# jianfenglihg/Unsupervised_depth_OpticalFlow_egomotion

Hardware: AMD Instinct MI355X
Metric: frame-pairs/sec (832x256, geom mode) (higher is better)
Workload: dtype f32; 1 GPU; train_step: mode=geom, 832x256, batch=4/GPU, num_scales=3, fwd+bwd+Adam; global_batch=4, parallelism=dp1, hw_queues=4, stream_priorities=auto

## Files before the change

### unsupervised_depth_opticalflow_egomotion_amd/csrc/ops_wino.hip

```cpp
#include "dfe_internal.h"
#include "dfe_mfma_stage.h"
#include "dfe_device.h"
#include <hip/hip_runtime.h>
#include <algorithm>
#include <cstdlib>

namespace dfe {


struct WinoEpi { const float* bias; float slope; float* y2; long y2bs; };
__device__ __forceinline__ float wino_act(float v, float bv, float slope) { v += bv; return v > 0.0f ? v : v * slope; }

#ifndef WINO_SCHED
#define WINO_SCHED 1
#endif
constexpr int WN_CC = 16;
constexpr int WN_XP = 20;

template <bool TRANSPOSED>
__device__ __forceinline__ void wino_weight_one(const float* __restrict__ w, float* __restrict__ U, int K, int C, int Kpad, int idx) {
  const int k = idx % Kpad, c = idx / Kpad;
  float g[9];
#pragma unroll
  for (int t = 0; t < 9; ++t) {
    float v = 0.0f;
    if (k < K) v = TRANSPOSED ? w[(static_cast<long>(c) * K + k) * 9 + 8 - t] : w[(static_cast<long>(k) * C + c) * 9 + t];
    g[t] = v;
  }
  float r[4][3];
#pragma unroll
  for (int j = 0; j < 3; ++j) {
    r[0][j] = g[j];
    r[1][j] = 0.5f * ((g[j] + g[3 + j]) + g[6 + j]);
    r[2][j] = 0.5f * ((g[j] - g[3 + j]) + g[6 + j]);
    r[3][j] = g[6 + j];
  }
  float* o = U + ((static_cast<long>(k >> 5) * C + c) * 32 + (k & 31)) * 16;
#pragma unroll
  for (int i = 0; i < 4; ++i) {
    o[i * 4 + 0] = r[i][0];
    o[i * 4 + 1] = 0.5f * ((r[i][0] + r[i][1]) + r[i][2]);
    o[i * 4 + 2] = 0.5f * ((r[i][0] - r[i][1]) + r[i][2]);
    o[i * 4 + 3] = r[i][2];
  }
}

template <bool TRANSPOSED>
__global__ void __launch_bounds__(256) k_wino_weights(const float* __restrict__ w, float* __restrict__ U, int K, int C, int Kpad) {
  const int idx = blockIdx.x * 256 + threadIdx.x;
  if (idx >= Kpad * C) return;
  wino_weight_one<TRANSPOSED>(w, U, K, C, Kpad, idx);
}

__global__ void __launch_bounds__(256) k_wino_weights_multi(const long* __restrict__ table, const int* __restrict__ blockmap) {
  const long* e = table + 6L * blockmap[blockIdx.x];
  const float* w = reinterpret_cast<const float*>(e[0]);
  float* U = reinterpret_cast<float*>(e[1]);
  const int K = static_cast<int>(e[2]), C = static_cast<int>(e[3]), Kpad = (K + 31) / 32 * 32;
  const int idx = (static_cast<int>(blockIdx.x) - static_cast<int>(e[5])) * 256 + threadIdx.x;
  if (idx >= Kpad * C) return;
  if (e[4]) wino_weight_one<true>(w, U, K, C, Kpad, idx);
  else wino_weight_one<false>(w, U, K, C, Kpad, idx);
}

__global__ void __launch_bounds__(256) k_wino_sum(const float* __restrict__ part, float* __restrict__ y, long ybs, int nsp, int B, long KHW,
                                                  long HWo, WinoEpi epi) {
  const long idx = static_cast<long>(blockIdx.x) * 256 + threadIdx.x;
  if (idx >= B * KHW) return;
  float s = part[idx];
  for (int k = 1; k < nsp; ++k) s += part[static_cast<long>(k) * B * KHW + idx];
  const long b = idx / KHW, r = idx - b * KHW;
  if (epi.bias || epi.slope != 1.0f) s = wino_act(s, epi.bias ? epi.bias[r / HWo] : 0.0f, epi.slope);
  y[b * ybs + r] = s;
  if (epi.y2) epi.y2[b * epi.y2bs + r] = s;
}

template <int PP, int NW, int NH>
__global__ void __launch_bounds__(64 * NW, 2) k_wino_fwd16(const float* __restrict__ x, const float* __restrict__ U, float* __restrict__ y,
                                                       long ybs, int B, int C, int K, int H, int W, int P, int TH, int TW, int ntiles,
                                                       unsigned nkt, int dil, unsigned nsp, int cps, float* __restrict__ part, WinoEpi epi,
                                                       unsigned nitems) {
  extern __shared__ float lds[];
  const int tid = threadIdx.x, lane = tid & 63, wv = tid >> 6, n = lane & 15, kq = lane >> 4;
  for (unsigned item = blockIdx.x; item < nitems; item += gridDim.x) {
  if (item != blockIdx.x) __syncthreads();
  const unsigned lid = xcd_swizzle(item, nitems);
  const int kt = static_cast<int>(lid % nkt), sp = static_cast<int>((lid / nkt) % nsp), tb = static_cast<int>(lid / (nkt * nsp));
  const int cbeg = sp * cps, Cend = min(C, cbeg + cps);
  const int Ho = H + 2 * P - 2, Wo = W + 2 * P - 2, HW = H * W;
  const int tile = min(tb * (16 * NW) + wv * 16 + n, ntiles - 1);
  int b, ty, tx, py = 0, px = 0;
  if (PP >= 0 || dil == 1) {
    b = tile / (TH * TW);
    const int tr = tile - b * TH * TW;
    ty = tr / TW; tx = tr - ty * TW;
  } else {
    const int per_row = TW * dil, per_phase = TH * per_row, per_img = per_phase * dil;
    b = tile / per_img;
    int tr = tile - b * per_img;
    py = tr / per_phase; tr -= py * per_phase;
    ty = tr / per_row; tr -= ty * per_row;
    tx = tr / dil; px = tr - tx * dil;
  }
  const int iy0 = 2 * ty - P, ix0 = 2 * tx - P;
  constexpr bool PAIR = PP >= 0;
  constexpr bool USE_L = PP == 1 || PP == 2, USE_R = PP == 1 || PP == 0;
  unsigned off[16], inb = 0;
  bool edge_l = false, edge_r = false;
  if (PAIR) {
    const bool okL = tx >= 1, okR = 2 * tx + 3 < W, okO = 2 * tx + 1 < W;
    edge_l = USE_L && okL && n == 0;
    edge_r = USE_R && okR && (n == 15 || tx == TW - 1);
#pragma unroll
    for (int i = 0; i < 4; ++i) {
      const int yy = iy0 + i;
      const bool ok = yy >= 0 && yy < H;
      const unsigned rowb = 4u * (static_cast<unsigned>(b) * C * HW + (ok ? yy * W : 0));
      off[i] = rowb + (okO ? 8u * static_cast<unsigned>(tx) : 0u);
      off[4 + i] = rowb + (edge_l ? 8u * static_cast<unsigned>(tx - 1) : edge_r ? 8u * static_cast<unsigned>(tx + 1) : 0u);
      off[8 + i] = 0; off[12 + i] = 0;
      inb |= ok ? (1u << i) : 0u;
    }
    inb |= (okL ? 16u : 0u) | (okR ? 32u : 0u) | (okO ? 64u : 0u);
  } else {
    const int Hq = H / dil, Wq = W / dil;
#pragma unroll
    for (int i = 0; i < 4; ++i)
#pragma unroll
      for (int j = 0; j < 4; ++j) {
        const int yy = iy0 + i, xx = ix0 + j;
        const bool ok = yy >= 0 && yy < Hq && xx >= 0 && xx < Wq;
        off[i * 4 + j] = 4u * (static_cast<unsigned>(b) * C * HW + (ok ? (py + dil * yy) * W + px + dil * xx : 0));
        inb |= ok ? (1u << (i * 4 + j)) : 0u;
      }
  }
  f32x4 acc[NH][16];
#pragma unroll
  for (int h = 0; h < NH; ++h)
#pragma unroll
    for (int s = 0; s < 16; ++s) acc[h][s] = f32x4{0.0f, 0.0f, 0.0f, 0.0f};
  const float* Ut = U + static_cast<long>(kt) * C * 512;
  const char* xc = reinterpret_cast<const char*>(x);
  float dn[16];
  unsigned mn;

  unsigned cbl = 4u * static_cast<unsigned>(cbeg + kq) * HW;
  const unsigned cstep = 16u * static_cast<unsigned>(HW);
  auto issue = [&](int c) {
    const bool cok = c < Cend;
    mn = cok ? inb : 0u;
    const unsigned cb = cok ? cbl : 0u;
    cbl += cstep;
    if (PAIR) {
#pragma unroll
      for (int i = 0; i < 4; ++i) {
        const f32x2 p = *reinterpret_cast<const f32x2*>(xc + (off[i] + cb));
        dn[2 * i] = p[0]; dn[2 * i + 1] = p[1];
      }
      if (edge_l || edge_r) {
#pragma unroll
        for (int i = 0; i < 4; ++i) {
          const f32x2 p = *reinterpret_cast<const f32x2*>(xc + (off[4 + i] + cb));
          dn[8 + 2 * i] = p[0]; dn[9 + 2 * i] = p[1];
        }
      }
    } else {
#pragma unroll
      for (int q = 0; q < 16; ++q) dn[q] = *reinterpret_cast<const float*>(xc + (off[q] + cb));
    }
  };
  auto shr1 = [](float v) { return __int_as_float(__builtin_amdgcn_update_dpp(0, __float_as_int(v), 0x111, 0xF, 0xF, true)); };
  auto shl1 = [](float v) { return __int_as_float(__builtin_amdgcn_update_dpp(0, __float_as_int(v), 0x101, 0xF, 0xF, true)); };
  constexpr unsigned NEED = 0xFu | (USE_L ? 16u : 0u) | (USE_R ? 32u : 0u) | 64u;
  const bool plain_wave = PAIR && __all(static_cast<int>((inb & NEED) == NEED)) != 0;
  auto gather = [&](float (&d)[16]) {
    if (PAIR && plain_wave && __all(static_cast<int>(mn != 0u)) != 0) {
#pragma unroll
      for (int i = 0; i < 4; ++i) {
        const float o1 = dn[2 * i], o2 = dn[2 * i + 1], e1 = dn[8 + 2 * i], e2 = dn[9 + 2 * i];
        float l1 = 0.0f, l2 = 0.0f, r1 = 0.0f, r2 = 0.0f;
        if (USE_L) {
          if (PP == 2) { l1 = shr1(o1); l1 = edge_l ? e1 : l1; }
          l2 = shr1(o2); l2 = edge_l ? e2 : l2;
        }
        if (USE_R) {
          r1 = shl1(o1); r1 = edge_r ? e1 : r1;
          if (PP == 0) { r2 = shl1(o2); r2 = edge_r ? e2 : r2; }
        }
        if (PP == 1) { d[4 * i] = l2; d[4 * i + 1] = o1; d[4 * i + 2] = o2; d[4 * i + 3] = r1; }
        else if (PP == 0) { d[4 * i] = o1; d[4 * i + 1] = o2; d[4 * i + 2] = r1; d[4 * i + 3] = r2; }
        else { d[4 * i] = l1; d[4 * i + 1] = l2; d[4 * i + 2] = o1; d[4 * i + 3] = o2; }
      }
    } else if (PAIR) {
#pragma unroll
      for (int i = 0; i < 4; ++i) {
        const bool rok = (mn >> i) & 1u;
        const bool oko = rok && (mn & 64u);
        const float o1 = oko ? dn[2 * i] : 0.0f, o2 = oko ? dn[2 * i + 1] : 0.0f;
        const float e1 = rok ? dn[8 + 2 * i] : 0.0f, e2 = rok ? dn[9 + 2 * i] : 0.0f;
        float l1 = 0.0f, l2 = 0.0f, r1 = 0.0f, r2 = 0.0f;
        if (USE_L) {
          if (PP == 2) l1 = shr1(o1);
          l2 = shr1(o2);
          if (PP == 2) l1 = (mn & 16u) ? (edge_l ? e1 : l1) : 0.0f;
          l2 = (mn & 16u) ? (edge_l ? e2 : l2) : 0.0f;
        }
        if (USE_R) {
          r1 = shl1(o1);
          if (PP == 0) r2 = shl1(o2);
          r1 = (mn & 32u) ? (edge_r ? e1 : r1) : 0.0f;
          if (PP == 0) r2 = (mn & 32u) ? (edge_r ? e2 : r2) : 0.0f;
        }
        if (PP == 1) { d[4 * i] = l2; d[4 * i + 1] = o1; d[4 * i + 2] = o2; d[4 * i + 3] = r1; }
        else if (PP == 0) { d[4 * i] = o1; d[4 * i + 1] = o2; d[4 * i + 2] = r1; d[4 * i + 3] = r2; }
        else { d[4 * i] = l1; d[4 * i + 1] = l2; d[4 * i + 2] = o1; d[4 * i + 3] = o2; }
      }
    } else {
#pragma unroll
      for (int q = 0; q < 16; ++q) d[q] = ((mn >> q) & 1u) ? dn[q] : 0.0f;
    }
  };
#pragma unroll
  for (int i = 8; i < 16; ++i) dn[i] = 0.0f;
  issue(cbeg + kq);
  constexpr int SC = 8, SLAB = SC * 32 * WN_XP;
  constexpr int NTH = 64 * NW;
  f32x4 wreg[SC * 128 / NTH];
  auto wfetch = [&](int c0) {
    const int nc = min(SC, Cend - c0);
#pragma unroll
    for (int i = 0; i < SC * 128 / NTH; ++i) {
      const int e = tid + i * NTH;
      wreg[i] = *reinterpret_cast<const f32x4*>(Ut + static_cast<long>(c0) * 512 + (e < nc * 128 ? e : 0) * 4);
    }
  };
  auto wstore = [&](float* buf) {
#pragma unroll
    for (int i = 0; i < SC * 128 / NTH; ++i) {
      const int e = tid + i * NTH;
      *reinterpret_cast<f32x4*>(buf + (e >> 2) * WN_XP + (e & 3) * 4) = wreg[i];
    }
  };
  wfetch(cbeg);
  wstore(lds);
  __syncthreads();
  int cur = 0;
  for (int c0 = cbeg; c0 < Cend; c0 += SC) {
    const int nc = min(SC, Cend - c0);
    const bool more = c0 + SC < Cend;
    if (more) wfetch(c0 + SC);
    const float* slab = lds + cur * SLAB;
    for (int cs = 0; cs < nc; cs += 4) {
      float d[16], t[16], v[16];
      const float* up = slab + (min(cs + kq, nc - 1) * 32 + n) * WN_XP;
      auto ldU = [&](int h, int q) { return *reinterpret_cast<const f32x4*>(up + h * 16 * WN_XP + 4 * q); };
      f32x4 ua, ub, uc;
      if (NH == 2 && WINO_SCHED) { ua = ldU(0, 0); ub = ldU(0, 1); __builtin_amdgcn_sched_barrier(0); }
      gather(d);
      issue(c0 + cs + 4 + kq);
#pragma unroll
      for (int j = 0; j < 4; ++j) {
        t[j] = d[j] - d[8 + j];
        t[4 + j] = d[4 + j] + d[8 + j];
        t[8 + j] = d[8 + j] - d[4 + j];
        t[12 + j] = d[4 + j] - d[12 + j];
      }
#pragma unroll
      for (int i = 0; i < 4; ++i) {
        v[i * 4 + 0] = t[i * 4] - t[i * 4 + 2];
        v[i * 4 + 1] = t[i * 4 + 1] + t[i * 4 + 2];
        v[i * 4 + 2] = t[i * 4 + 2] - t[i * 4 + 1];
        v[i * 4 + 3] = t[i * 4 + 1] - t[i * 4 + 3];
      }
      if (NH == 2 && WINO_SCHED) {
        auto mfma4 = [&](int h, int q, const f32x4& u) {
#pragma unroll
          for (int j = 0; j < 4; ++j) acc[h][4 * q + j] = __builtin_amdgcn_mfma_f32_16x16x4f32(u[j], v[4 * q + j], acc[h][4 * q + j], 0, 0, 0);
        };
        __builtin_amdgcn_sched_barrier(0);
        uc = ldU(0, 2);
        mfma4(0, 0, ua); ua = ldU(0, 3);
        mfma4(0, 1, ub); ub = ldU(1, 0);
        mfma4(0, 2, uc); uc = ldU(1, 1);
        mfma4(0, 3, ua); ua = ldU(1, 2);
        mfma4(1, 0, ub); ub = ldU(1, 3);
        mfma4(1, 1, uc);
        mfma4(1, 2, ua);
        mfma4(1, 3, ub);
#define SGB_DS(n) __builtin_amdgcn_sched_group_barrier(0x100, n, 0)
#define SGB_MFMA(n) __builtin_amdgcn_sched_group_barrier(0x008, n, 0)
        SGB_DS(1); SGB_MFMA(4); SGB_DS(1); SGB_MFMA(4); SGB_DS(1); SGB_MFMA(4); SGB_DS(1); SGB_MFMA(4); SGB_DS(1); SGB_MFMA(4); SGB_DS(1); SGB_MFMA(12);
#undef SGB_DS
#undef SGB_MFMA
        __builtin_amdgcn_sched_barrier(0);
        continue;
      }
#pragma unroll
      for (int h = 0; h < NH; ++h) {
        float u[16];
#pragma unroll
        for (int q = 0; q < 4; ++q) {
          const f32x4 w4 = *reinterpret_cast<const f32x4*>(up + h * 16 * WN_XP + 4 * q);
          u[4 * q] = w4[0]; u[4 * q + 1] = w4[1]; u[4 * q + 2] = w4[2]; u[4 * q + 3] = w4[3];
        }
#pragma unroll
        for (int s = 0; s < 16; ++s) acc[h][s] = __builtin_amdgcn_mfma_f32_16x16x4f32(u[s], v[s], acc[h][s], 0, 0, 0);
      }
    }
    if (more) {
      wstore(lds + (cur ^ 1) * SLAB);
      __syncthreads();
      cur ^= 1;
    }
  }
  if (tb * (16 * NW) + wv * 16 + n >= ntiles) continue;
  const int Hoq = (PP >= 0 || dil == 1) ? Ho : H / dil, Woq = (PP >= 0 || dil == 1) ? Wo : W / dil;
  const int oy = 2 * ty, ox = 2 * tx;
  const int sy = dil * Wo, sx = dil;
  const long kplane = static_cast<long>(Ho) * Wo;
  const long ooff = static_cast<long>(py + dil * oy) * Wo + px + dil * ox;
  float* yb = (nsp > 1 ? part + (static_cast<long>(sp) * B + b) * K * kplane : y + b * ybs) + ooff;
  const bool fused = nsp == 1 && (epi.bias != nullptr || epi.slope != 1.0f);
  float* y2b = (nsp == 1 && epi.y2) ? epi.y2 + b * epi.y2bs + ooff : nullptr;
  const bool even_w = dil == 1 && (Wo & 1) == 0;
  const bool pair_st = even_w && (reinterpret_cast<uintptr_t>(nsp > 1 ? part : y) & 7) == 0 && ((nsp > 1 ? 0 : ybs) & 1) == 0;
  const bool pair_st2 = even_w && y2b && (reinterpret_cast<uintptr_t>(epi.y2) & 7) == 0 && (epi.y2bs & 1) == 0;
#pragma unroll
  for (int h = 0; h < NH; ++h)
#pragma unroll
    for (int r = 0; r < 4; ++r) {
      const int k = kt * 32 + 16 * h + 4 * kq + r;
      if (k >= K) continue;
      float t0[4], t1[4];
#pragma unroll
      for (int s = 0; s < 4; ++s) {
        t0[s] = (acc[h][s][r] + acc[h][4 + s][r]) + acc[h][8 + s][r];
        t1[s] = (acc[h][4 + s][r] - acc[h][8 + s][r]) - acc[h][12 + s][r];
      }
      float y00 = (t0[0] + t0[1]) + t0[2], y01 = (t0[1] - t0[2]) - t0[3];
      float y10 = (t1[0] + t1[1]) + t1[2], y11 = (t1[1] - t1[2]) - t1[3];
      if (fused) {
        const float bv = epi.bias ? epi.bias[k] : 0.0f;
        y00 = wino_act(y00, bv, epi.slope); y01 = wino_act(y01, bv, epi.slope);
        y10 = wino_act(y10, bv, epi.slope); y11 = wino_act(y11, bv, epi.slope);
      }
      float* o = yb + static_cast<long>(k) * Ho * Wo;
      if (pair_st) {
        if (ox < Woq) {
          if (oy < Hoq) *reinterpret_cast<f32x2*>(o) = f32x2{y00, y01};
          if (oy + 1 < Hoq) *reinterpret_cast<f32x2*>(o + sy) = f32x2{y10, y11};
        }
      } else {
        if (oy < Hoq) {
          if (ox < Woq) o[0] = y00;
          if (ox + 1 < Woq) o[sx] = y01;
        }
        if (oy + 1 < Hoq) {
          if (ox < Woq) o[sy] = y10;
          if (ox + 1 < Woq) o[sy + sx] = y11;
        }
      }
      if (y2b) {
        float* o2 = y2b + static_cast<long>(k) * Ho * Wo;
        if (pair_st2) {
          if (ox < Woq) {
            if (oy < Hoq) *reinterpret_cast<f32x2*>(o2) = f32x2{y00, y01};
            if (oy + 1 < Hoq) *reinterpret_cast<f32x2*>(o2 + sy) = f32x2{y10, y11};
          }
        } else {
          if (oy < Hoq) {
            if (ox < Woq) o2[0] = y00;
            if (ox + 1 < Woq) o2[sx] = y01;
          }
          if (oy + 1 < Hoq) {
            if (ox < Woq) o2[sy] = y10;
            if (ox + 1 < Woq) o2[sy + sx] = y11;
          }
        }
      }
    }
  }
}

}

using namespace dfe;

static int wn_dims(int B, int Ci, int Co, int H, int W, int P) {
  if (B <= 0 || Ci <= 0 || Co <= 0 || H <= 0 || W <= 0) return DFE_ERR_DIMS;
  if (P < 0 || P > 2) return DFE_ERR_UNSUPPORTED;
  if (H + 2 * P < 3 || W + 2 * P < 3) return DFE_ERR_DIMS;
  if (static_cast<long>(B) * Ci * H * W >= (1L << 30) || static_cast<long>(Co) * H * W >= (1L << 31) || Co > 65535 * 32) return DFE_ERR_DIMS;
  return DFE_OK;
}

extern "C" long dfe_wino_weight_floats(int Ci, int Co) { return (Ci <= 0 || Co <= 0) ? 0 : static_cast<long>((Co + 31) / 32) * 32 * Ci * 16; }

extern "C" long dfe_wino_weight_floats(int Ci, int Co);

struct WinoSplit { int nsp, cps; long part_floats; };

static WinoSplit wino_split(long ntiles, int Kpad, int Ci, int B, int Co, int Ho, int Wo) {
  WinoSplit w{1, Ci, 0};
  static const bool enabled = env_int("DFE_WINO_SPLIT", 1) != 0;
  const long nblk = (ntiles + 63) / 64 * (Kpad / 32);
  if (!enabled || nblk >= 384 || Ci < 64) return w;
  int nsp = static_cast<int>((512 + nblk - 1) / nblk);
  nsp = std::min(nsp, std::min(Ci / 32, 8));
  if (nsp < 2) return w;
  w.cps = ((Ci + nsp - 1) / nsp + 7) / 8 * 8;
  w.nsp = (Ci + w.cps - 1) / w.cps;
  if (w.nsp < 2) { w.nsp = 1; w.cps = Ci; return w; }
  w.part_floats = static_cast<long>(w.nsp) * B * Co * Ho * Wo;
  return w;
}

static int wino_run(const float* x, const float* weight, float* y, long y_batch_stride, float* wbuf, float* part, long part_floats, int B,
                    int Ci, int Co, int H, int W, int P, int dil, int transposed_weight, void* stream, WinoEpi epi = WinoEpi{nullptr, 1.0f, nullptr, 0}) {
  if (!x || !y || !wbuf) return DFE_ERR_NULL;
  const int rc = wn_dims(B, Ci, Co, H, W, P);
  if (rc != DFE_OK) return rc;
  if (dil < 1 || (dil > 1 && (P != 1 || H % dil != 0 || W % dil != 0 || H / dil < 2 || W / dil < 2))) return DFE_ERR_UNSUPPORTED;
  const int Ho = dil > 1 ? H : H + 2 * P - 2, Wo = dil > 1 ? W : W + 2 * P - 2;
  if (y_batch_stride < static_cast<long>(Co) * Ho * Wo || (epi.y2 && epi.y2bs < static_cast<long>(Co) * Ho * Wo)) return DFE_ERR_DIMS;
  if ((reinterpret_cast<uintptr_t>(wbuf) & 15) != 0) return DFE_ERR_UNSUPPORTED;
  if (part && (reinterpret_cast<uintptr_t>(part) & 15) != 0) return DFE_ERR_UNSUPPORTED;
  hipStream_t st = static_cast<hipStream_t>(stream);
  const int Kpad = (Co + 31) / 32 * 32;
  const int nw = Kpad * Ci;
  if (weight) {
    if (transposed_weight) k_wino_weights<true><<<(nw + 255) / 256, 256, 0, st>>>(weight, wbuf, Co, Ci, Kpad);
    else k_wino_weights<false><<<(nw + 255) / 256, 256, 0, st>>>(weight, wbuf, Co, Ci, Kpad);
    DFE_LAUNCH_CHECK();
  }
  const int TH = (Ho / dil + 1) / 2, TW = (Wo / dil + 1) / 2;
  const long ntiles = static_cast<long>(B) * TH * TW * dil * dil;
  if (ntiles >= (1L << 31)) return DFE_ERR_DIMS;
  const size_t lds_bytes = sizeof(float) * WN_CC * 32 * WN_XP;
  {
    const unsigned nkt = Kpad / 32;
    WinoSplit sp = wino_split(ntiles, Kpad, Ci, B, Co, Ho, Wo);
    if (dil > 1 || !part || part_floats < sp.part_floats) sp = WinoSplit{1, Ci, 0};
    const int tpb = 64;
    const long nblk = (ntiles + tpb - 1) / tpb * nkt * sp.nsp;
    if (nblk >= (1L << 31)) return DFE_ERR_DIMS;
    static const bool pair_ok = env_int("DFE_WINO_PAIR", 1) != 0;
    const bool pair = pair_ok && dil == 1 && W % 2 == 0 && (reinterpret_cast<uintptr_t>(x) & 7) == 0;
    const unsigned nitems = static_cast<unsigned>(nblk);
    static const int persist = env_int("DFE_WINO_PERSIST", 0);
    const unsigned g = persist > 0 ? std::min(nitems, static_cast<unsigned>(persist)) : nitems;
    const int nt = static_cast<int>(ntiles);
    const int pp = pair ? P : -1;
#define WN_LAUNCH(PPV, NHV) k_wino_fwd16<PPV, 4, NHV><<<g, 256, lds_bytes, st>>>(x, wbuf, y, y_batch_stride, B, Ci, Co, H, W, P, TH, TW, nt, nkt, dil, static_cast<unsigned>(sp.nsp), sp.cps, part, epi, nitems)
    if (Co <= 16) {
      if (pp == 1) WN_LAUNCH(1, 1); else if (pp == 0) WN_LAUNCH(0, 1); else if (pp == 2) WN_LAUNCH(2, 1); else WN_LAUNCH(-1, 1);
    } else {
      if (pp == 1) WN_LAUNCH(1, 2); else if (pp == 0) WN_LAUNCH(0, 2); else if (pp == 2) WN_LAUNCH(2, 2); else WN_LAUNCH(-1, 2);
    }
#undef WN_LAUNCH
    DFE_LAUNCH_CHECK();
    if (sp.nsp > 1) {
      const long khw = static_cast<long>(Co) * Ho * Wo, n = B * khw;
      k_wino_sum<<<static_cast<unsigned>((n + 255) / 256), 256, 0, st>>>(part, y, y_batch_stride, sp.nsp, B, khw, static_cast<long>(Ho) * Wo, epi);
    }
  }
  DFE_LAUNCH_CHECK();
  return DFE_OK;
}

extern "C" long dfe_wino_scratch_floats(int B, int Ci, int Co, int H, int W, int P) {
  if (B <= 0 || Ci <= 0 || Co <= 0 || H <= 0 || W <= 0 || P < 0 || P > 2) return 0;
  const int Ho = H + 2 * P - 2, Wo = W + 2 * P - 2;
  if (Ho < 1 || Wo < 1) return 0;
  const int Kpad = (Co + 31) / 32 * 32;
  const long ntiles = static_cast<long>(B) * ((Ho + 1) / 2) * ((Wo + 1) / 2);
  return static_cast<long>(Kpad) * Ci * 16 + wino_split(ntiles, Kpad, Ci, B, Co, Ho, Wo).part_floats;
}

extern "C" int dfe_wino_conv3x3(const float* x, const float* weight, float* y, long y_batch_stride, float* wbuf, long wbuf_floats, int B,
                                int Ci, int Co, int H, int W, int P, int transposed_weight, void* stream) {
  if (!weight) return DFE_ERR_NULL;
  const long ufl = dfe_wino_weight_floats(Ci, Co);
  if (wbuf_floats < ufl) return DFE_ERR_WORKSPACE;
  return wino_run(x, weight, y, y_batch_stride, wbuf, wbuf ? wbuf + ufl : nullptr, wbuf_floats - ufl, B, Ci, Co, H, W, P, 1, transposed_weight, stream);
}

extern "C" int dfe_wino_conv3x3_dilated(const float* x, const float* weight, float* y, long y_batch_stride, float* wbuf, int B,
                                        int Ci, int Co, int H, int W, int dilation, int transposed_weight, void* stream) {
  if (!weight) return DFE_ERR_NULL;
  return wino_run(x, weight, y, y_batch_stride, wbuf, nullptr, 0, B, Ci, Co, H, W, 1, dilation, transposed_weight, stream);
}

extern "C" int dfe_wino_conv3x3_u(const float* x, const float* U, float* y, long y_batch_stride, float* part, long part_floats, int B, int Ci,
                                  int Co, int H, int W, int P, int dilation, void* stream) {
  return wino_run(x, nullptr, y, y_batch_stride, const_cast<float*>(U), part, part_floats, B, Ci, Co, H, W, dilation > 1 ? 1 : P, dilation, 0,
                  stream);
}

extern "C" int dfe_wino_conv3x3_u_act(const float* x, const float* U, const float* bias, float slope, float* y, long y_batch_stride, float* y2,
                                      long y2_batch_stride, float* part, long part_floats, int B, int Ci, int Co, int H, int W, int P,
                                      int dilation, void* stream) {
  return wino_run(x, nullptr, y, y_batch_stride, const_cast<float*>(U), part, part_floats, B, Ci, Co, H, W, dilation > 1 ? 1 : P, dilation, 0,
                  stream, WinoEpi{bias, slope, y2, y2_batch_stride});
}

extern "C" long dfe_wino_transform_blocks(int Ci, int Co) {
  if (Ci <= 0 || Co <= 0) return 0;
  return (static_cast<long>((Co + 31) / 32 * 32) * Ci + 255) / 256;
}

extern "C" int dfe_wino_transform_weights_multi(const long* table, const int* blockmap, int n_blocks, void* stream) {
  if (!table || !blockmap) return DFE_ERR_NULL;
  if (n_blocks <= 0) return DFE_ERR_DIMS;
  k_wino_weights_multi<<<n_blocks, 256, 0, static_cast<hipStream_t>(stream)>>>(table, blockmap);
  DFE_LAUNCH_CHECK();
  return DFE_OK;
}
```

Before: 434.1 frame-pairs/s.

## Use buffer loads with OOB offsets and restructure Winograd channel loop pipeline

Replaces global loads in the Winograd forward kernel with raw buffer loads whose out-of-bounds offsets (a sentinel value) return zero in hardware, removing the per-element mask selects in the gather. The edge/zero handling via DPP now uses the old-value operand, and a wave-uniform 'inner' flag skips fixups for interior waves. The channel loop is restructured into a two-step-per-slab software pipeline with explicit placement of the next input load and LDS weight store between the transform halves. It adds complexity and relies on buffer OOB semantics, and it tightens the dimension limit accordingly.

```diff
diff --git a/unsupervised_depth_opticalflow_egomotion_amd/csrc/ops_wino.hip b/unsupervised_depth_opticalflow_egomotion_amd/csrc/ops_wino.hip
--- a/unsupervised_depth_opticalflow_egomotion_amd/csrc/ops_wino.hip
+++ b/unsupervised_depth_opticalflow_egomotion_amd/csrc/ops_wino.hip
@@ -16,6 +16,8 @@
 #endif
 constexpr int WN_CC = 16;
 constexpr int WN_XP = 20;
+constexpr unsigned WN_OOB = 0xfffffff0u;
+typedef unsigned u32x2 __attribute__((ext_vector_type(2)));
 
 template <bool TRANSPOSED>
 __device__ __forceinline__ void wino_weight_one(const float* __restrict__ w, float* __restrict__ U, int K, int C, int Kpad, int idx) {
@@ -82,6 +84,7 @@
                                                        unsigned nitems) {
   extern __shared__ float lds[];
   const int tid = threadIdx.x, lane = tid & 63, wv = tid >> 6, n = lane & 15, kq = lane >> 4;
+  const float* up0 = lds + (kq * 32 + n) * WN_XP;
   for (unsigned item = blockIdx.x; item < nitems; item += gridDim.x) {
   if (item != blockIdx.x) __syncthreads();
   const unsigned lid = xcd_swizzle(item, nitems);
@@ -105,23 +108,24 @@
   const int iy0 = 2 * ty - P, ix0 = 2 * tx - P;
   constexpr bool PAIR = PP >= 0;
   constexpr bool USE_L = PP == 1 || PP == 2, USE_R = PP == 1 || PP == 0;
-  unsigned off[16], inb = 0;
-  bool edge_l = false, edge_r = false;
+  constexpr int NV = PAIR ? 8 : 16;
+  unsigned vo[NV];
+  bool zl = false, zr = false;
+  const unsigned lane0 = 4u * (static_cast<unsigned>(b) * C + kq) * HW;
   if (PAIR) {
     const bool okL = tx >= 1, okR = 2 * tx + 3 < W, okO = 2 * tx + 1 < W;
-    edge_l = USE_L && okL && n == 0;
-    edge_r = USE_R && okR && (n == 15 || tx == TW - 1);
+    const bool edge_l = USE_L && okL && n == 0;
+    const bool edge_r = USE_R && okR && (n == 15 || tx == TW - 1);
+    zl = USE_L && !okL && n != 0;
+    zr = USE_R && n != 15 && (PP == 0 ? edge_r : !okR);
 #pragma unroll
     for (int i = 0; i < 4; ++i) {
       const int yy = iy0 + i;
       const bool ok = yy >= 0 && yy < H;
-      const unsigned rowb = 4u * (static_cast<unsigned>(b) * C * HW + (ok ? yy * W : 0));
-      off[i] = rowb + (okO ? 8u * static_cast<unsigned>(tx) : 0u);
-      off[4 + i] = rowb + (edge_l ? 8u * static_cast<unsigned>(tx - 1) : edge_r ? 8u * static_cast<unsigned>(tx + 1) : 0u);
-      off[8 + i] = 0; off[12 + i] = 0;
-      inb |= ok ? (1u << i) : 0u;
-    }
-    inb |= (okL ? 16u : 0u) | (okR ? 32u : 0u) | (okO ? 64u : 0u);
+      const unsigned rowb = lane0 + 4u * static_cast<unsigned>(ok ? yy * W : 0);
+      vo[i] = ok && okO ? rowb + 8u * static_cast<unsigned>(tx) : WN_OOB;
+      vo[4 + i] = ok && edge_l ? rowb + 8u * static_cast<unsigned>(tx - 1) : ok && edge_r ? rowb + 8u * static_cast<unsigned>(tx + 1) : WN_OOB;
+    }
   } else {
     const int Hq = H / dil, Wq = W / dil;
 #pragma unroll
@@ -130,99 +134,90 @@
       for (int j = 0; j < 4; ++j) {
         const int yy = iy0 + i, xx = ix0 + j;
         const bool ok = yy >= 0 && yy < Hq && xx >= 0 && xx < Wq;
-        off[i * 4 + j] = 4u * (static_cast<unsigned>(b) * C * HW + (ok ? (py + dil * yy) * W + px + dil * xx : 0));
-        inb |= ok ? (1u << (i * 4 + j)) : 0u;
-      }
-  }
+        vo[i * 4 + j] = ok ? lane0 + 4u * static_cast<unsigned>((py + dil * yy) * W + px + dil * xx) : WN_OOB;
+      }
+  }
+  const int inner = PAIR ? __builtin_amdgcn_readfirstlane(static_cast<int>(__builtin_amdgcn_ballot_w64(zl || zr) != 0ull)) : 0;
   f32x4 acc[NH][16];
 #pragma unroll
   for (int h = 0; h < NH; ++h)
 #pragma unroll
     for (int s = 0; s < 16; ++s) acc[h][s] = f32x4{0.0f, 0.0f, 0.0f, 0.0f};
   const float* Ut = U + static_cast<long>(kt) * C * 512;
-  const char* xc = reinterpret_cast<const char*>(x);
+  const int ns = (Cend - cbeg + 3) >> 2;
   float dn[16];
-  unsigned mn;
-
-  unsigned cbl = 4u * static_cast<unsigned>(cbeg + kq) * HW;
-  const unsigned cstep = 16u * static_cast<unsigned>(HW);
-  auto issue = [&](int c) {
-    const bool cok = c < Cend;
-    mn = cok ? inb : 0u;
-    const unsigned cb = cok ? cbl : 0u;
-    cbl += cstep;
+
+  const char* xs = reinterpret_cast<const char*>(x) + 4L * cbeg * HW;
+  const long cstep = 16L * HW;
+  const int nrec = static_cast<int>(4u * static_cast<unsigned>(B) * C * HW);
+  const bool past = cbeg + 4 * (ns - 1) + kq >= Cend;
+  auto issue = [&](bool last) {
+    const __amdgpu_buffer_rsrc_t xr = __builtin_amdgcn_make_buffer_rsrc(const_cast<char*>(xs), 0, nrec, 0x00020000);
+    xs += cstep;
+    auto loads = [&]() {
+      if (PAIR) {
+#pragma unroll
+        for (int q = 0; q < 8; ++q) {
+          const u32x2 p = __builtin_amdgcn_raw_buffer_load_b64(xr, vo[q], 0, 0);
+          dn[2 * q] = __uint_as_float(p[0]); dn[2 * q + 1] = __uint_as_float(p[1]);
+        }
+      } else {
+#pragma unroll
+        for (int q = 0; q < 16; ++q) dn[q] = __uint_as_float(__builtin_amdgcn_raw_buffer_load_b32(xr, vo[q], 0, 0));
+      }
+    };
+    if (last) {
+#pragma unroll
+      for (int q = 0; q < 16; ++q) dn[q] = 0.0f;
+      if (!past) loads();
+    } else {
+      loads();
+    }
+  };
+  auto shr1 = [](float old, float v) { return __int_as_float(__builtin_amdgcn_update_dpp(__float_as_int(old), __float_as_int(v), 0x111, 0xF, 0xF, false)); };
+  auto shl1 = [](float old, float v) { return __int_as_float(__builtin_amdgcn_update_dpp(__float_as_int(old), __float_as_int(v), 0x101, 0xF, 0xF, false)); };
+  auto gather = [&](float (&d)[16]) {
     if (PAIR) {
-#pragma unroll
-      for (int i = 0; i < 4; ++i) {
-        const f32x2 p = *reinterpret_cast<const f32x2*>(xc + (off[i] + cb));
-        dn[2 * i] = p[0]; dn[2 * i + 1] = p[1];
-      }
-      if (edge_l || edge_r) {
-#pragma unroll
-        for (int i = 0; i < 4; ++i) {
-          const f32x2 p = *reinterpret_cast<const f32x2*>(xc + (off[4 + i] + cb));
-          dn[8 + 2 * i] = p[0]; dn[9 + 2 * i] = p[1];
-        }
-      }
-    } else {
-#pragma unroll
-      for (int q = 0; q < 16; ++q) dn[q] = *reinterpret_cast<const float*>(xc + (off[q] + cb));
-    }
-  };
-  auto shr1 = [](float v) { return __int_as_float(__builtin_amdgcn_update_dpp(0, __float_as_int(v), 0x111, 0xF, 0xF, true)); };
-  auto shl1 = [](float v) { return __int_as_float(__builtin_amdgcn_update_dpp(0, __float_as_int(v), 0x101, 0xF, 0xF, true)); };
-  constexpr unsigned NEED = 0xFu | (USE_L ? 16u : 0u) | (USE_R ? 32u : 0u) | 64u;
-  const bool plain_wave = PAIR && __all(static_cast<int>((inb & NEED) == NEED)) != 0;
-  auto gather = [&](float (&d)[16]) {
-    if (PAIR && plain_wave && __all(static_cast<int>(mn != 0u)) != 0) {
+      float l1[4], l2[4], r1[4], r2[4], k1[4], k2[4];
 #pragma unroll
       for (int i = 0; i < 4; ++i) {
         const float o1 = dn[2 * i], o2 = dn[2 * i + 1], e1 = dn[8 + 2 * i], e2 = dn[9 + 2 * i];
-        float l1 = 0.0f, l2 = 0.0f, r1 = 0.0f, r2 = 0.0f;
+        l1[i] = l2[i] = r1[i] = r2[i] = 0.0f;
+        k1[i] = PP == 0 ? e1 : 0.0f; k2[i] = PP == 0 ? e2 : 0.0f;
         if (USE_L) {
-          if (PP == 2) { l1 = shr1(o1); l1 = edge_l ? e1 : l1; }
-          l2 = shr1(o2); l2 = edge_l ? e2 : l2;
+          if (PP == 2) l1[i] = shr1(e1, o1);
+          l2[i] = shr1(e2, o2);
         }
         if (USE_R) {
-          r1 = shl1(o1); r1 = edge_r ? e1 : r1;
-          if (PP == 0) { r2 = shl1(o2); r2 = edge_r ? e2 : r2; }
-        }
-        if (PP == 1) { d[4 * i] = l2; d[4 * i + 1] = o1; d[4 * i + 2] = o2; d[4 * i + 3] = r1; }
-        else if (PP == 0) { d[4 * i] = o1; d[4 * i + 1] = o2; d[4 * i + 2] = r1; d[4 * i + 3] = r2; }
-        else { d[4 * i] = l1; d[4 * i + 1] = l2; d[4 * i + 2] = o1; d[4 * i + 3] = o2; }
-      }
-    } else if (PAIR) {
+          r1[i] = shl1(e1, o1);
+          if (PP == 0) r2[i] = shl1(e2, o2);
+        }
+      }
+      if (inner) {
+#pragma unroll
+        for (int i = 0; i < 4; ++i) {
+          if (USE_L) {
+            if (PP == 2) l1[i] = zl ? 0.0f : l1[i];
+            l2[i] = zl ? 0.0f : l2[i];
+          }
+          if (USE_R) {
+            r1[i] = zr ? k1[i] : r1[i];
+            if (PP == 0) r2[i] = zr ? k2[i] : r2[i];
+          }
+        }
+      }
 #pragma unroll
       for (int i = 0; i < 4; ++i) {
-        const bool rok = (mn >> i) & 1u;
-        const bool oko = rok && (mn & 64u);
-        const float o1 = oko ? dn[2 * i] : 0.0f, o2 = oko ? dn[2 * i + 1] : 0.0f;
-        const float e1 = rok ? dn[8 + 2 * i] : 0.0f, e2 = rok ? dn[9 + 2 * i] : 0.0f;
-        float l1 = 0.0f, l2 = 0.0f, r1 = 0.0f, r2 = 0.0f;
-        if (USE_L) {
-          if (PP == 2) l1 = shr1(o1);
-          l2 = shr1(o2);
-          if (PP == 2) l1 = (mn & 16u) ? (edge_l ? e1 : l1) : 0.0f;
-          l2 = (mn & 16u) ? (edge_l ? e2 : l2) : 0.0f;
-        }
-        if (USE_R) {
-          r1 = shl1(o1);
-          if (PP == 0) r2 = shl1(o2);
-          r1 = (mn & 32u) ? (edge_r ? e1 : r1) : 0.0f;
-          if (PP == 0) r2 = (mn & 32u) ? (edge_r ? e2 : r2) : 0.0f;
-        }
-        if (PP == 1) { d[4 * i] = l2; d[4 * i + 1] = o1; d[4 * i + 2] = o2; d[4 * i + 3] = r1; }
-        else if (PP == 0) { d[4 * i] = o1; d[4 * i + 1] = o2; d[4 * i + 2] = r1; d[4 * i + 3] = r2; }
-        else { d[4 * i] = l1; d[4 * i + 1] = l2; d[4 * i + 2] = o1; d[4 * i + 3] = o2; }
+        const float o1 = dn[2 * i], o2 = dn[2 * i + 1];
+        if (PP == 1) { d[4 * i] = l2[i]; d[4 * i + 1] = o1; d[4 * i + 2] = o2; d[4 * i + 3] = r1[i]; }
+        else if (PP == 0) { d[4 * i] = o1; d[4 * i + 1] = o2; d[4 * i + 2] = r1[i]; d[4 * i + 3] = r2[i]; }
+        else { d[4 * i] = l1[i]; d[4 * i + 1] = l2[i]; d[4 * i + 2] = o1; d[4 * i + 3] = o2; }
       }
     } else {
 #pragma unroll
-      for (int q = 0; q < 16; ++q) d[q] = ((mn >> q) & 1u) ? dn[q] : 0.0f;
+      for (int q = 0; q < 16; ++q) d[q] = dn[q];
     }
   };
-#pragma unroll
-  for (int i = 8; i < 16; ++i) dn[i] = 0.0f;
-  issue(cbeg + kq);
   constexpr int SC = 8, SLAB = SC * 32 * WN_XP;
   constexpr int NTH = 64 * NW;
   f32x4 wreg[SC * 128 / NTH];
@@ -241,74 +236,88 @@
       *reinterpret_cast<f32x4*>(buf + (e >> 2) * WN_XP + (e & 3) * 4) = wreg[i];
     }
   };
-  wfetch(cbeg);
-  wstore(lds);
-  __syncthreads();
-  int cur = 0;
-  for (int c0 = cbeg; c0 < Cend; c0 += SC) {
-    const int nc = min(SC, Cend - c0);
-    const bool more = c0 + SC < Cend;
-    if (more) wfetch(c0 + SC);
-    const float* slab = lds + cur * SLAB;
-    for (int cs = 0; cs < nc; cs += 4) {
-      float d[16], t[16], v[16];
-      const float* up = slab + (min(cs + kq, nc - 1) * 32 + n) * WN_XP;
-      auto ldU = [&](int h, int q) { return *reinterpret_cast<const f32x4*>(up + h * 16 * WN_XP + 4 * q); };
-      f32x4 ua, ub, uc;
-      if (NH == 2 && WINO_SCHED) { ua = ldU(0, 0); ub = ldU(0, 1); __builtin_amdgcn_sched_barrier(0); }
-      gather(d);
-      issue(c0 + cs + 4 + kq);
-#pragma unroll
-      for (int j = 0; j < 4; ++j) {
-        t[j] = d[j] - d[8 + j];
-        t[4 + j] = d[4 + j] + d[8 + j];
-        t[8 + j] = d[8 + j] - d[4 + j];
-        t[12 + j] = d[4 + j] - d[12 + j];
-      }
-#pragma unroll
-      for (int i = 0; i < 4; ++i) {
-        v[i * 4 + 0] = t[i * 4] - t[i * 4 + 2];
-        v[i * 4 + 1] = t[i * 4 + 1] + t[i * 4 + 2];
-        v[i * 4 + 2] = t[i * 4 + 2] - t[i * 4 + 1];
-        v[i * 4 + 3] = t[i * 4 + 1] - t[i * 4 + 3];
-      }
-      if (NH == 2 && WINO_SCHED) {
-        auto mfma4 = [&](int h, int q, const f32x4& u) {
-#pragma unroll
-          for (int j = 0; j < 4; ++j) acc[h][4 * q + j] = __builtin_amdgcn_mfma_f32_16x16x4f32(u[j], v[4 * q + j], acc[h][4 * q + j], 0, 0, 0);
-        };
-        __builtin_amdgcn_sched_barrier(0);
-        uc = ldU(0, 2);
-        mfma4(0, 0, ua); ua = ldU(0, 3);
-        mfma4(0, 1, ub); ub = ldU(1, 0);
-        mfma4(0, 2, uc); uc = ldU(1, 1);
-        mfma4(0, 3, ua); ua = ldU(1, 2);
-        mfma4(1, 0, ub); ub = ldU(1, 3);
-        mfma4(1, 1, uc);
-        mfma4(1, 2, ua);
-        mfma4(1, 3, ub);
+  auto step = [&](const float* up, auto between) {
+    float d[16], t[16], v[16];
+    auto ldU = [&](int h, int q) { return *reinterpret_cast<const f32x4*>(up + h * 16 * WN_XP + 4 * q); };
+    f32x4 ua, ub, uc;
+    if (NH == 2 && WINO_SCHED) { ua = ldU(0, 0); ub = ldU(0, 1); __builtin_amdgcn_sched_barrier(0); }
+    gather(d);
+#pragma unroll
+    for (int j = 0; j < 4; ++j) {
+      t[j] = d[j] - d[8 + j];
+      t[4 + j] = d[4 + j] + d[8 + j];
+      t[8 + j] = d[8 + j] - d[4 + j];
+      t[12 + j] = d[4 + j] - d[12 + j];
+    }
+    if (PAIR) __builtin_amdgcn_sched_barrier(0);
+    between();
+#pragma unroll
+    for (int i = 0; i < 4; ++i) {
+      v[i * 4 + 0] = t[i * 4] - t[i * 4 + 2];
+      v[i * 4 + 1] = t[i * 4 + 1] + t[i * 4 + 2];
+      v[i * 4 + 2] = t[i * 4 + 2] - t[i * 4 + 1];
+      v[i * 4 + 3] = t[i * 4 + 1] - t[i * 4 + 3];
+    }
+    if (NH == 2 && WINO_SCHED) {
+      auto mfma4 = [&](int h, int q, const f32x4& u) {
+#pragma unroll
+        for (int j = 0; j < 4; ++j) acc[h][4 * q + j] = __builtin_amdgcn_mfma_f32_16x16x4f32(u[j], v[4 * q + j], acc[h][4 * q + j], 0, 0, 0);
+      };
+      __builtin_amdgcn_sched_barrier(0);
+      uc = ldU(0, 2);
+      mfma4(0, 0, ua); ua = ldU(0, 3);
+      mfma4(0, 1, ub); ub = ldU(1, 0);
+      mfma4(0, 2, uc); uc = ldU(1, 1);
+      mfma4(0, 3, ua); ua = ldU(1, 2);
+      mfma4(1, 0, ub); ub = ldU(1, 3);
+      mfma4(1, 1, uc);
+      mfma4(1, 2, ua);
+      mfma4(1, 3, ub);
 #define SGB_DS(n) __builtin_amdgcn_sched_group_barrier(0x100, n, 0)
 #define SGB_MFMA(n) __builtin_amdgcn_sched_group_barrier(0x008, n, 0)
-        SGB_DS(1); SGB_MFMA(4); SGB_DS(1); SGB_MFMA(4); SGB_DS(1); SGB_MFMA(4); SGB_DS(1); SGB_MFMA(4); SGB_DS(1); SGB_MFMA(4); SGB_DS(1); SGB_MFMA(12);
+      SGB_DS(1); SGB_MFMA(4); SGB_DS(1); SGB_MFMA(4); SGB_DS(1); SGB_MFMA(4); SGB_DS(1); SGB_MFMA(4); SGB_DS(1); SGB_MFMA(4); SGB_DS(1); SGB_MFMA(12);
 #undef SGB_DS
 #undef SGB_MFMA
-        __builtin_amdgcn_sched_barrier(0);
-        continue;
-      }
-#pragma unroll
-      for (int h = 0; h < NH; ++h) {
-        float u[16];
-#pragma unroll
-        for (int q = 0; q < 4; ++q) {
-          const f32x4 w4 = *reinterpret_cast<const f32x4*>(up + h * 16 * WN_XP + 4 * q);
-          u[4 * q] = w4[0]; u[4 * q + 1] = w4[1]; u[4 * q + 2] = w4[2]; u[4 * q + 3] = w4[3];
-        }
-#pragma unroll
-        for (int s = 0; s < 16; ++s) acc[h][s] = __builtin_amdgcn_mfma_f32_16x16x4f32(u[s], v[s], acc[h][s], 0, 0, 0);
-      }
-    }
-    if (more) {
+      __builtin_amdgcn_sched_barrier(0);
+      return;
+    }
+#pragma unroll
+    for (int h = 0; h < NH; ++h) {
+      float u[16];
+#pragma unroll
+      for (int q = 0; q < 4; ++q) {
+        const f32x4 w4 = *reinterpret_cast<const f32x4*>(up + h * 16 * WN_XP + 4 * q);
+        u[4 * q] = w4[0]; u[4 * q + 1] = w4[1]; u[4 * q + 2] = w4[2]; u[4 * q + 3] = w4[3];
+      }
+#pragma unroll
+      for (int s = 0; s < 16; ++s) acc[h][s] = __builtin_amdgcn_mfma_f32_16x16x4f32(u[s], v[s], acc[h][s], 0, 0, 0);
+    }
+  };
+  wfetch(cbeg);
+  issue(ns == 1);
+  wstore(lds);
+  if (ns > 2) wfetch(cbeg + SC);
+  __syncthreads();
+  int s = 0, cur = 0;
+  for (; s + 3 < ns; s += 2) {
+    const float* up = up0 + cur * SLAB;
+    step(up, [&]() { issue(false); });
+    step(up + 4 * 32 * WN_XP, [&]() {
       wstore(lds + (cur ^ 1) * SLAB);
+      if (s + 4 < ns) wfetch(cbeg + 4 * s + 2 * SC);
+      issue(false);
+    });
+    __syncthreads();
+    cur ^= 1;
+  }
+  for (; s < ns; ++s) {
+    const int cs = 4 * (s & 1), nc = Cend - (cbeg + 4 * (s & ~1));
+    const bool fin = s + 1 == ns, turn = cs != 0 && !fin;
+    step(fin ? lds + cur * SLAB + (min(cs + kq, nc - 1) * 32 + n) * WN_XP : up0 + cur * SLAB + cs * 32 * WN_XP, [&]() {
+      if (turn) wstore(lds + (cur ^ 1) * SLAB);
+      if (!fin) issue(s + 2 == ns);
+    });
+    if (turn) {
       __syncthreads();
       cur ^= 1;
     }
@@ -390,7 +399,7 @@
   if (B <= 0 || Ci <= 0 || Co <= 0 || H <= 0 || W <= 0) return DFE_ERR_DIMS;
   if (P < 0 || P > 2) return DFE_ERR_UNSUPPORTED;
   if (H + 2 * P < 3 || W + 2 * P < 3) return DFE_ERR_DIMS;
-  if (static_cast<long>(B) * Ci * H * W >= (1L << 30) || static_cast<long>(Co) * H * W >= (1L << 31) || Co > 65535 * 32) return DFE_ERR_DIMS;
+  if (static_cast<long>(B) * Ci * H * W > WN_OOB / 4 || static_cast<long>(Co) * H * W >= (1L << 31) || Co > 65535 * 32) return DFE_ERR_DIMS;
   return DFE_OK;
 }
 
```

New measurement: 452.2 frame-pairs/s (median of 6 runs). +4.2%, better.
